# stresearch/xfr

Measured on AMD Instinct MI355X. Metric: triplet-contrastive-EBP saliency maps/sec, ResNet-101 224x224, higher is better.
Workload: dtype f32

## Files before the change

### xfr_amd/csrc/conv_gemm.hip

```cpp
#include <algorithm>
#include <atomic>
#include <mutex>
#include <vector>
#include "common.h"
#include <cstdio>
#include <cstdlib>

#include "conv_gemm_dev.h"
#include "conv_gemm_host.h"

std::atomic<long> g_conv_chain_launches[2];

namespace {

#ifndef XFR_MFM_WAVES
#define XFR_MFM_WAVES 6
#endif
#ifndef XFR_DUAL_WAVES
#define XFR_DUAL_WAVES 4
#endif
template <int TCO, int TM, int BK, int NST, int MODE, bool RELU, int CHAIN>
__global__ __launch_bounds__(NT, CHAIN == 0 ? 1 : (CHAIN == 1 ? 7 : (CHAIN == 4 ? XFR_DUAL_WAVES : XFR_MFM_WAVES))) void conv_gemm_kernel(const ConvParams p, const int n_co_tiles, const int n_m_tiles)
{
    constexpr bool ROW = TCO == 32;
// ... 673 lines not shown
        return &conv_gemm_ks_kernel<BK, NST, MODE, decltype(relu)::value, decltype(chain)::value>;
    });
}

template <int BK>
bool ks_ok(const ConvParams& p)
{
    if ((p.Cin % BK) != 0) return false;
    if (p.kh == 1 && p.kw == 1) return p.pad == 0 && p.stride <= 2;
    if (p.out_stride != 1) return false;
    return p.stride == 1 && p.tap_major == 1 && p.kh * p.kw <= 64;
}

bool is_vec_1x1(const ConvParams& p)
{
    return p.kh == 1 && p.kw == 1 && p.stride == 1 && p.pad == 0 && (p.M % 4) == 0 && p.OH == p.H && p.OW == p.W;
}

template <int BK, int NST>
bool launch_cfg_ks(const ConvParams& p, hipStream_t s)
{
    if (is_vec_1x1(p)) return launch_one_ks<BK, NST, MODE_VEC>(p, s);
    return launch_one_ks<BK, NST, MODE_TAP>(p, s);
}

template <int TCO, int TM, int BK, int NST>
bool launch_cfg(const ConvParams& p_in, hipStream_t s)
{
    ConvParams p = p_in;
    if (p.dualacc && p.kh == 1 && p.kw == 1 && p.tap_major == 0 && (p.Cin % 16) == 0) p.tap_major = 1;
    if (is_vec_1x1(p)) return launch_one<TCO, TM, BK, NST, MODE_VEC>(p, s);
    if (p.tap_major == 2) return launch_one<64, 64, 16, 4, MODE_TAP4>(p, s);
    if (p.tap_major && (p.Cin % BK) == 0) return launch_one<TCO, TM, BK, NST, MODE_TAP>(p, s);
    if (p.tap_major) return launch_one<TCO, TM, 16, 4, MODE_TAP>(p, s);
    return launch_one<TCO, TM, 16, 4, MODE_GEN>(p, s);
}

}

int conv_gemm_num_cus() { return num_cus(); }
int conv_gemm_plan_chain(ConvParams& q) { return plan_chain(q); }
void conv_gemm_warn_interpreted(const ConvParams& q) { warn_interpreted(q); }

int conv_gemm_chain_sig(const EwChain& ch)
{
    uint16_t codes[XFR_MAX_EW_STEPS];
    const int n = ew_chain_codes(ch, codes);
    if (n <= 0) return -1;
    for (int sgi = 0; sgi < kNumChainSigs; ++sgi) {
        bool same = true;
        for (int i = 0; i < XFR_MAX_EW_STEPS && same; ++i) same = kChainSigs[sgi][i] == (i < n ? codes[i] : 0);
        if (same) return sgi;
    }
    return -1;
}
int conv_gemm_num_chain_sigs() { return kNumChainSigs; }

int conv_gemm_cannot_launch(const ConvParams& p)
{
    if (p.chain.n <= 0) return 0;
    ConvParams q = p;
    return plan_chain(q);
}
const char* conv_gemm_refusal(int why)
{
    switch (why) {
        case 0: return "the convolution launch was refused without a reason";
        case 1: return "a dual (W / relu(W)) convolution launch carries a fused chain without a compiled epilogue";
        case 3: return "lean probe-forward steps and the dual-accumulator launch (ConvParams::dualacc) only exist together, behind a compiled epilogue";
        case 2: return "a fused chain with a MaxFeatureMap step (pair maximum / fan-out VJP) has no compiled epilogue and the interpreter does not run those steps";
        default: return "unknown convolution launch refusal";
    }
}

void conv_gemm_chain_launch_counts(long* compiled, long* interpreted)
{
    if (compiled) *compiled = g_conv_chain_launches[0].load();
    if (interpreted) *interpreted = g_conv_chain_launches[1].load();
}

static int pick_cfg_impl(const ConvParams& p_in, bool allow_split)
{
    ConvParams p = p_in;
    if (p.dualacc) { p.nhalves = 2; p.dualacc = 0; const int c = pick_cfg_impl(p, false); return c == CFG_ROW32 ? CFG_K16 : c; }
    if (allow_split && p.split_ok && conv_gemm_split_wanted(p)) return CFG_BF16X6;
    {
        const int rem = p.CoutTot % 64;
#ifndef XFR_NO_ROW_TILE
        if (rem > 0 && rem <= 32 && p.tap_major != 2 && p.out_stride == 1 && p.CoutTot > 32 && p.M > 64) return CFG_ROW32;
#endif
    }
    if (ks_ok<8>(p)) {
        if (p.kh == 1 && (p.stride == 2 || p.out_stride == 2 || p.as_strided)) return CFG_KS_4_4;
        if ((p.kh > 1 && p.K >= 2048) || (p.kh == 1 && (p.K == 512 || p.K >= 2048))) return CFG_KS_4_4;
    }
    const long tiles = (long)((p.CoutTot + 63) / 64) * p.nhalves * ((p.M + 63) / 64);
    if (p.K >= 1024 && tiles <= 512 && (p.tap_major ? (p.Cin % 32 == 0) : true)) return CFG_K32;
    return CFG_K16;
}
int conv_gemm_pick_cfg(const ConvParams& p_in) { return pick_cfg_impl(p_in, true); }

namespace {
struct LogRec { void* stream; int cout, nhalves, K, M, kh, chain, cfg, parts; };
std::mutex g_tune_mu;
std::atomic<int> g_tuning{0};
unsigned long long* g_stamps = nullptr;
int g_stamps_cap = 0;
int g_stamp_regions = 0, g_stamp_seq = 0;
unsigned long long* g_log = nullptr;
int g_log_cap = 0;
std::vector<LogRec> g_log_recs;
thread_local int g_last_cfg = 0;
constexpr size_t NO_LOG = (size_t)-1;

size_t tune_begin(ConvParams& p, hipStream_t s)
{
    p.stamps = nullptr;
    p.stamps_cap = 0;
    p.stamp_regions = 0;
    p.stamp_seq = 0;
    p.span = nullptr;
    size_t log_idx = NO_LOG;
    if (g_tuning.load(std::memory_order_relaxed)) {
        std::lock_guard<std::mutex> lk(g_tune_mu);
        p.stamps = g_stamps;
        p.stamps_cap = g_stamps_cap;
        p.stamp_regions = g_stamp_regions;
        p.stamp_seq = g_stamps ? g_stamp_seq++ : 0;
        if (g_log && (int)g_log_recs.size() < g_log_cap) {
            p.span = g_log + 8 * g_log_recs.size();
            log_idx = g_log_recs.size();
            g_log_recs.push_back(LogRec{(void*)s, p.CoutTot, p.dualacc ? 2 : p.nhalves, p.K, p.M, p.kh, p.chain.n, -1, 1});
        }
    }
    return log_idx;
}
void tune_ran(size_t log_idx, int cfg, int parts = 1)
{
    g_last_cfg = cfg;
    if (log_idx == NO_LOG) return;
    std::lock_guard<std::mutex> lk(g_tune_mu);
    if (log_idx < g_log_recs.size()) { g_log_recs[log_idx].cfg = cfg; g_log_recs[log_idx].parts = parts; }
}
int cfg_remap(int cfg)
{
    struct Remap { int v[32]; };
    static const Remap remap = [] {
        Remap r;
        for (int i = 0; i < 32; ++i) r.v[i] = i;
        if (const char* e = getenv("XFR_CFG_REMAP")) {
            int a = 0, b = 0, n = 0;
            while (sscanf(e, "%d:%d%n", &a, &b, &n) == 2) {
                if (a >= 0 && a < 32 && b >= 0 && b < 32) r.v[a] = b;
                e += n;
                if (*e == ',') ++e;
            }
        }
        return r;
    }();
    return (cfg >= 0 && cfg < 32) ? remap.v[cfg] : cfg;
}
}

void conv_gemm_set_stamps(unsigned long long* dev_ptr, int capacity_workgroups)
{
    std::lock_guard<std::mutex> lk(g_tune_mu);
// ... 51 lines not shown
```

### xfr_amd/csrc/conv_gemm_split.hip

```cpp
#include <algorithm>
#include <atomic>
#include <mutex>
#include <unordered_map>
#include <cstdio>
#include <cstdlib>
#include <type_traits>
#include "conv_gemm_dev.h"
#include "conv_gemm_host.h"

namespace {

typedef __bf16 v8bf __attribute__((ext_vector_type(8)));
typedef unsigned v4u __attribute__((ext_vector_type(4)));
constexpr int SP_T = 128, SP_BK = 16;
constexpr int SP_A_BYTES = 3 * 2 * SP_T * 16, SP_B_BYTES = 3 * 2 * SP_T * 16;
constexpr size_t SP_LDS = 3 * (size_t)(SP_A_BYTES + SP_B_BYTES);

typedef float v2f_t __attribute__((ext_vector_type(2)));
typedef __bf16 v2bf_t __attribute__((ext_vector_type(2)));
__device__ __forceinline__ unsigned cvt_pk_bf16(float lo, float hi)
{
    const v2f_t t = {lo, hi};
    return __builtin_bit_cast(unsigned, __builtin_convertvector(t, v2bf_t));
}
__device__ __forceinline__ void split_pair(float a, float b, unsigned& p0, unsigned& p1, unsigned& p2)
{
    p0 = cvt_pk_bf16(a, b);
    const float ra = a - __uint_as_float(p0 << 16), rb = b - __uint_as_float(p0 & 0xffff0000u);
    p1 = cvt_pk_bf16(ra, rb);
    const float sa = ra - __uint_as_float(p1 << 16), sb = rb - __uint_as_float(p1 & 0xffff0000u);
    p2 = cvt_pk_bf16(sa, sb);
}

constexpr int SPP_MAX_HALO = 64, SPP_MAX_TAPS = 25;

__host__ __device__ inline int spp_halo(const ConvParams& p) { return p.pad * p.W + p.pad; }
__host__ __device__ inline int spp_patch_len(const ConvParams& p) { return SP_T + 2 * spp_halo(p); }
inline size_t spp_lds_bytes(const ConvParams& p) { return (size_t)3 * SP_A_BYTES + (size_t)2 * 6 * (spp_patch_len(p) + 1) * 16; }

constexpr int NT8 = 512;

template <int N>
__device__ __forceinline__ void sp8_wait_barrier()
{
    asm volatile("s_waitcnt vmcnt(%0) lgkmcnt(0)\n\ts_barrier" ::"n"(N) : "memory");
}

template <bool RELU, int CHAIN, bool PATCH>
__global__ __launch_bounds__(NT8, 2) void conv_gemm_split_kernel(const ConvParams p, const uint16_t* __restrict__ ws0, const uint16_t* __restrict__ ws1,
                                                                  const int n_co_tiles, const int n_m_tiles)
{
    extern __shared__ __attribute__((aligned(16))) float smem[];
    unsigned char* lds = reinterpret_cast<unsigned char*>(smem);
    constexpr int NST = 3, D = NST - 1, XBASE = NST * SP_A_BYTES;
    const int tid = threadIdx.x, lane = tid & 63, wave8 = __builtin_amdgcn_readfirstlane(tid >> 6);
    const int wr4 = wave8 >> 1, wc = wave8 & 1;
    const int l31 = lane & 31, lhi = lane >> 5;
    const bool two_dma = wave8 < 4;
    if (wave8 < 4) stamp(p, wave8, lane, 0, 4);

    const int nparts = p.tail_s > 1 ? p.tail_s : 1;
    const int tile_lin = nparts > 1 ? (int)blockIdx.x / nparts : (int)blockIdx.x;
    const int part = (int)blockIdx.x - tile_lin * nparts;
    const int lid = xcd_remap(tile_lin, n_co_tiles * n_m_tiles);
    const int tile_m = lid / n_co_tiles;
    const int tile_co_all = lid - tile_m * n_co_tiles;
    const int n_co_half = n_co_tiles / p.nhalves;
    const int half = tile_co_all / n_co_half;
    const int tile_co = tile_co_all - half * n_co_half;
    const int co0 = tile_co * SP_T, m0 = tile_m * SP_T;
    const uint16_t* __restrict__ wsel = half ? ws1 : ws0;
    const float* __restrict__ bsel = half ? p.bias_pos : p.bias;
    float* __restrict__ osel = half ? p.out1 : p.out0;
    const int T = p.kh * p.kw, ncb = p.Cin / SP_BK, nk = p.K / SP_BK;
    const int units = PATCH ? ncb : (nk + 2) / 3, ustep = PATCH ? T : 3;
    const int ubase = units / nparts, urem = units - ubase * nparts;
    const int u0 = part * ubase + min(part, urem), u1 = u0 + ubase + (part < urem ? 1 : 0);
    const int k0 = u0 * ustep, k_end = min(u1 * ustep, nk);
    const int halo = spp_halo(p), PL = spp_patch_len(p);
    const int PS = PATCH ? (PL + 1) * 16 : SP_T * 16;
    const int XB = 6 * PS;
    const unsigned chan_bytes = (unsigned)p.in_nb * p.H * p.W * 4u;
    const __amdgpu_buffer_rsrc_t rW = __builtin_amdgcn_make_buffer_rsrc((void*)wsel, 0, n_co_half * nk * SP_A_BYTES, 0x00020000);
    const __amdgpu_buffer_rsrc_t rIn = __builtin_amdgcn_make_buffer_rsrc((void*)p.in, 0, (int)p.in_bytes, 0x00020000);
    const unsigned lds_base = (unsigned)(size_t)(__attribute__((address_space(3))) unsigned char*)(lds);

    unsigned t_voff = OOB, t_lds = 0;
    bool t_ok = false;
    int base_m = 0;
    unsigned long long tapmask = 0ull;
    const int sm = tid & 127, skq = wave8 >> 1;
    if constexpr (PATCH) {
        const int kh_ = tid >= PL ? 1 : 0, q = tid - kh_ * PL;
        const long g = (long)m0 - halo + q;
        t_ok = tid < 2 * PL;
        const bool in_row = t_ok && g >= 0 && g < (long)p.in_nb * p.H * p.W;
        t_voff = in_row ? (unsigned)g * 4u + (unsigned)(kh_ * 8) * chan_bytes : OOB;
        t_lds = lds_base + XBASE + kh_ * PS + q * 16;
    } else {
        const int m = m0 + sm;
        const bool m_ok = m < p.M;
        const int mm = m_ok ? m : 0;
        const int ohw = p.OH * p.OW;
        const int n = mm / ohw;
        const int r = mm - n * ohw;
        const int oh = r / p.OW;
        const int ow = r - oh * p.OW;
        const int ih0 = oh * p.stride - p.pad, iw0 = ow * p.stride - p.pad - p.pad_dw;
        base_m = n * p.H * p.W + ih0 * p.W + iw0;
        if (m_ok) {
            unsigned long long vw = 0ull;
            for (int dw = 0; dw < p.kw; ++dw)
                if ((unsigned)(iw0 + dw) < (unsigned)p.W) vw |= 1ull << dw;
            for (int dh = 0; dh < p.kh; ++dh)
                if ((unsigned)(ih0 + dh) < (unsigned)p.H) tapmask |= vw << (dh * p.kw);
        }
        t_lds = lds_base + XBASE + ((skq >> 1) * SP_T + sm) * 16 + (skq & 1) * 8;
    }
    int c_pos[2] = {0, 0};
    unsigned c_mask[2] = {0u, 0u};
    if constexpr (PATCH) {
#pragma unroll
        for (int j = 0; j < 2; ++j) {
            const int c = wc * 64 + j * 32 + l31, m = m0 + c;
            c_pos[j] = c + halo;
            unsigned mk = 0u;
            if (m < p.M) {
                const int ohw = p.OH * p.OW;
                const int r = m % ohw;
                const int oh = r / p.OW, ow = r - oh * p.OW;
                for (int dh = 0; dh < p.kh; ++dh)
                    for (int dw = 0; dw < p.kw; ++dw)
                        if ((unsigned)(oh + dh - p.pad) < (unsigned)p.H && (unsigned)(ow + dw - p.pad) < (unsigned)p.W) mk |= 1u << (dh * p.kw + dw);
            }
            c_mask[j] = mk;
        }
    }
    const unsigned char* a_lane = lds + (lhi * SP_T + wr4 * 32 + l31) * 16;
    const unsigned char* b_plane = lds + XBASE + lhi * PS;

    v16f acc[2], pipe[2];
#pragma unroll
    for (int j = 0; j < 2; ++j)
#pragma unroll
        for (int r = 0; r < 16; ++r) { acc[j][r] = 0.f; pipe[j][r] = 0.f; }

    auto dma = [&](int kt, int stage, int ch) {
        __builtin_amdgcn_raw_ptr_buffer_load_lds(rW, (lptr_t)(lds + stage * SP_A_BYTES + ch * 1024), 16, (ch * 1024 + lane * 16) | (kt < k_end ? 0u : OOB),
                                                 (tile_co * nk + kt) * SP_A_BYTES, 0, 0);
    };
    auto load_w = [&](int kt, int stage) {
        dma(kt, stage, wave8);
        if (two_dma) dma(kt, stage, 8 + wave8);
    };
    auto fold = [&](bool negated) {
        if (negated) { acc[0] -= pipe[0]; acc[1] -= pipe[1]; }
        else { acc[0] += pipe[0]; acc[1] += pipe[1]; }
    };
    auto mfmas = [&](const v8bf (&af)[3], const v8bf (&bf)[3][2], auto FIRST) {
        constexpr int TA[6] = {2, 1, 0, 1, 0, 0}, TB[6] = {0, 1, 2, 0, 1, 0};
        v16f zero;
#pragma unroll
        for (int r = 0; r < 16; ++r) zero[r] = 0.f;
#pragma unroll
        for (int t = 0; t < 6; ++t)
#pragma unroll
            for (int j = 0; j < 2; ++j)
                pipe[j] = __builtin_amdgcn_mfma_f32_32x32x16_bf16(af[TA[t]], bf[TB[t]][j], (t == 0 && decltype(FIRST)::value) ? zero : pipe[j], 0, 0, 0);
    };
    std::integral_constant<int, 0> S0; std::integral_constant<int, 1> S1; std::integral_constant<int, 2> S2;
    std::integral_constant<bool, true> first; std::integral_constant<bool, false> later;

    if constexpr (PATCH) {
        float xp[8];
        auto load_patch = [&](int cb) {
            const unsigned so = (unsigned)(cb * SP_BK) * chan_bytes;
#pragma unroll
            for (int i = 0; i < 8; ++i) xp[i] = __uint_as_float(__builtin_amdgcn_raw_buffer_load_b32(rIn, t_voff, so + (unsigned)i * chan_bytes, 0));
        };
        auto store_patch = [&](int buf, unsigned flip) {
            v4u q0, q1, q2;
#pragma unroll
            for (int i = 0; i < 4; ++i) {
                const float a = RELU ? fmaxf(xp[2 * i], 0.f) : xp[2 * i], b = RELU ? fmaxf(xp[2 * i + 1], 0.f) : xp[2 * i + 1];
                unsigned h0, h1, h2;
                split_pair(a, b, h0, h1, h2);
                q0[i] = h0 ^ flip; q1[i] = h1 ^ flip; q2[i] = h2 ^ flip;
            }
            if (t_ok) {
                const unsigned at = t_lds + buf * XB;
                asm volatile("ds_write_b128 %0, %1" :: "v"(at), "v"(q0));
                asm volatile("ds_write_b128 %0, %1" :: "v"(at + 2 * PS), "v"(q1));
                asm volatile("ds_write_b128 %0, %1" :: "v"(at + 4 * PS), "v"(q2));
            }
        };
        int tap = 0, cb = u0, buf = 0, shift = -halo, tdw = 0;
        bool xl_prev = false, xl_now = false;
        const bool mfma_first = wave8 < 4;
        auto load_part = [&](int kt, v8bf (&af)[3], v8bf (&bf)[3][2]) {
            const int st1 = (kt + 1) % 3, st3 = kt % 3;
            const bool more = cb + 1 < u1;
            xl_now = false;
            if (more && tap == 2) store_patch(buf ^ 1, ((cb + 1) & 1) ? 0x80008000u : 0u);
            load_w(k0 + kt + 3, kt < 0 ? 2 : st3);
            if (more && tap == 0) { load_patch(cb + 1); xl_now = true; }
            const unsigned char* As = a_lane + (kt < 0 ? 0 : st1) * SP_A_BYTES;
#pragma unroll
            for (int pc = 0; pc < 3; ++pc) af[pc] = *(const v8bf*)(As + pc * 2 * SP_T * 16);
#pragma unroll
            for (int j = 0; j < 2; ++j) {
                const int pos = ((c_mask[j] >> tap) & 1u) ? c_pos[j] + shift : PL;
                const unsigned char* Bs = b_plane + buf * XB + pos * 16;
#pragma unroll
                for (int pc = 0; pc < 3; ++pc) bf[pc][j] = *(const v8bf*)(Bs + pc * 2 * PS);
            }
            tap += 1; tdw += 1; shift += 1;
            if (tdw == p.kw) { tdw = 0; shift += p.W - p.kw; }
            if (tap == T) { tap = 0; shift = -halo; cb += 1; buf ^= 1; }
        };
        auto end_step = [&]() {
            if (xl_now || xl_prev) { if (two_dma) sp8_wait_barrier<10>(); else sp8_wait_barrier<9>(); }
            else { if (two_dma) sp8_wait_barrier<2>(); else sp8_wait_barrier<1>(); }
            xl_prev = xl_now;
        };
        auto step = [&](int kt, v8bf (&caf)[3], v8bf (&cbf)[3][2], v8bf (&naf)[3], v8bf (&nbf)[3][2], auto FIRST) {
            if (mfma_first) mfmas(caf, cbf, FIRST);
            __builtin_amdgcn_sched_barrier(0);
            load_part(kt, naf, nbf);
            __builtin_amdgcn_sched_barrier(0);
            if (!mfma_first) mfmas(caf, cbf, FIRST);
            end_step();
        };
        if (tid < 12) {
            const v4u z = {0u, 0u, 0u, 0u};
            asm volatile("ds_write_b128 %0, %1" :: "v"(lds_base + XBASE + (tid / 6) * XB + (tid % 6) * PS + PL * 16), "v"(z));
        }
        if (u1 - u0 == 1) {
            const v4u z = {0u, 0u, 0u, 0u};
            for (int i = tid; i < 6 * (PL + 1); i += NT8) asm volatile("ds_write_b128 %0, %1" :: "v"(lds_base + XBASE + XB + i * 16), "v"(z));
        }
        load_w(k0, 0);
        load_w(k0 + 1, 1);
        load_patch(u0);
        asm volatile("s_waitcnt vmcnt(0)" ::: "memory");
        store_patch(0, (u0 & 1) ? 0x80008000u : 0u);
        sp8_wait_barrier<0>();
        v8bf f0a[3], f0b[3][2], f1a[3], f1b[3][2];
        load_part(-1, f0a, f0b);
        end_step();
        if (wave8 < 4) stamp(p, wave8, lane, 1);
        int pass_in_blk = 0;
// ... 51 lines not shown
            load_w(kt + D, stD);
            load_x(kt + 3, xnew);
            const unsigned char* As = a_lane + wst * SP_A_BYTES;
            const unsigned char* Bs = b_plane + st * XB + (wc * 64 + l31) * 16;
            v8bf af[3], bf[3][2];
#pragma unroll
            for (int pc = 0; pc < 3; ++pc) {
                af[pc] = *(const v8bf*)(As + pc * 2 * SP_T * 16);
#pragma unroll
                for (int j = 0; j < 2; ++j) bf[pc][j] = *(const v8bf*)(Bs + pc * 2 * PS + j * 32 * 16);
            }
            mfmas(af, bf, FIRST);
            store_x(xcur, st1, flip);
            if (two_dma) sp8_wait_barrier<8 + 2 * (D - 1)>(); else sp8_wait_barrier<8 + (D - 1)>();
            wst = wst + 1 == NST ? 0 : wst + 1;
        };
        float x0[4], x1[4], x2[4];
        unsigned flip = (u0 & 1) ? 0x80008000u : 0u;
        load_w(k0, 0);
        load_x(k0, x0);
        asm volatile("s_waitcnt vmcnt(0)" ::: "memory");
        store_x(x0, 0, flip);
#pragma unroll
        for (int d = 1; d < D; ++d) load_w(k0 + d, d);
        load_x(k0 + 1, x0);
        load_x(k0 + 2, x1);
        if (two_dma) sp8_wait_barrier<8 + 2 * (D - 1)>(); else sp8_wait_barrier<8 + (D - 1)>();
        if (wave8 < 4) stamp(p, wave8, lane, 1);
        for (int kt = k0; kt < k_end; kt += 3) {
            const bool negated = flip != 0u;
            step(kt, S0, x0, x2, flip, first);
            step(kt + 1, S1, x1, x0, flip, later);
            flip ^= 0x80008000u;
            step(kt + 2, S2, x2, x1, flip, later);
            fold(negated);
        }
    }
    wait_vmcnt<0>();
    asm volatile("s_waitcnt lgkmcnt(0)" ::: "memory");
    if (wave8 < 4) stamp(p, wave8, lane, 2);

    if (nparts > 1) {
        constexpr int TILE_FLOATS = SP_T * SP_T;
        float* __restrict__ slab = p.tail_ws + ((long)tile_lin * nparts + part) * TILE_FLOATS + tid;
#pragma unroll
        for (int j = 0; j < 2; ++j)
#pragma unroll
            for (int r = 0; r < 16; ++r) __hip_atomic_store(slab + (j * 16 + r) * NT8, acc[j][r], __ATOMIC_RELAXED, __HIP_MEMORY_SCOPE_AGENT);
        wait_vmcnt<0>();
        __syncthreads();
        int* flag = reinterpret_cast<int*>(smem);
        if (tid == 0) {
            const unsigned old = atomicAdd(p.tail_cnt + tile_lin, 1u);
            const int last = (old == (unsigned)(nparts - 1));
            if (last) atomicExch(p.tail_cnt + tile_lin, 0u);
            *flag = last;
        }
        __syncthreads();
        const int last_part = *flag;
        __syncthreads();
        if (!last_part) {
            if (wave8 < 4) { stamp(p, wave8, lane, 3); stamp(p, wave8, lane, 4); }
            return;
        }
        const float* __restrict__ src = p.tail_ws + (long)tile_lin * nparts * TILE_FLOATS + tid;
#pragma unroll
        for (int j = 0; j < 2; ++j)
#pragma unroll
            for (int r = 0; r < 16; ++r) acc[j][r] = 0.f;
        for (int q = 0; q < nparts; ++q, src += TILE_FLOATS) {
            float v[32];
#pragma unroll
            for (int r = 0; r < 32; ++r) v[r] = __hip_atomic_load(src + r * NT8, __ATOMIC_RELAXED, __HIP_MEMORY_SCOPE_AGENT);
#pragma unroll
            for (int r = 0; r < 32; ++r) acc[r >> 4][r & 15] += v[r];
        }
    }
    if (wave8 < 4) stamp(p, wave8, lane, 3);

#pragma unroll 1
    for (int c = 0; c < 2; ++c) {
        v16f t = acc[0];
        const int wq = (wr4 & 1) * 2 + c;
        block_epilogue<CHAIN>(p, t, smem + (wave8 - wq) * (32 * 36), tid & 255, lane, wq, co0 + (wr4 >> 1) * 64, m0 + wc * 64, half, -1, 0, 1, osel, bsel, nullptr);
        acc[0] = acc[1];
    }
    if (wave8 < 4) stamp(p, wave8, lane, 4);
}

__global__ void split_pack_kernel(const float* __restrict__ w, uint16_t* __restrict__ planes, int K, int cout, int ldw, int taps)
{
    const long idx = (long)blockIdx.x * blockDim.x + threadIdx.x;
    if (idx >= (long)K * cout) return;
    const int k = (int)(idx / cout), co = (int)(idx - (long)k * cout);
    unsigned h[3];
    split_pair(w[(long)k * ldw + co], 0.f, h[0], h[1], h[2]);
    const int cin = K / taps, tap = k / cin, ci = k - tap * cin;
    const int rt = co / SP_T, r = co - rt * SP_T, kt = (ci / SP_BK) * taps + tap, kk = ci % SP_BK, nk = K / SP_BK;
#pragma unroll
    for (int q = 0; q < 3; ++q)
        planes[((((long)(rt * nk + kt) * 3 + q) * 2 + kk / 8) * SP_T + r) * 8 + kk % 8] = (uint16_t)(h[q] & 0xffffu);
}

struct SplitPack { uint16_t* planes; int K, cout, ldw, taps; };
static std::mutex g_split_mu;
static std::unordered_map<const float*, SplitPack> g_split;

bool split_patch_ok(const ConvParams& p)
{
    const int T = p.kh * p.kw;
    if (T < 5 || T > SPP_MAX_TAPS || (T % 3) != 0 || p.stride != 1 || p.tap_major != 1) return false;
    if (p.OH != p.H || p.OW != p.W || 2 * p.pad != p.kh - 1 || 2 * p.pad != p.kw - 1 || p.pad_dw != 0) return false;
    static const bool off = getenv("XFR_SPLIT_NO_PATCH") != nullptr;
    return spp_halo(p) <= SPP_MAX_HALO && !off;
}

bool split_can_run(const ConvParams& p)
{
    if (p.dualacc || p.out_stride != 1 || p.as_strided || p.co_pair > 0 || p.stride != 1) return false;
    if ((p.Cin % SP_BK) != 0 || (p.K % SP_BK) != 0 || (p.CoutTot % SP_T) != 0) return false;
    if (p.kh == 1 && p.kw == 1) return p.pad == 0;
    return p.tap_major == 1 && p.kh * p.kw <= 64;
}
struct SplitPolicy { int min_k1, min_k3, min_tiles, min_hw, max_parts, min_steps, min_cb, parts_below_hw; };
const SplitPolicy& split_policy()
{
    static const SplitPolicy pol = [] {
        SplitPolicy q{256, 1152, 128, 49, 2, 32, 4, 196};
        if (const char* e = getenv("XFR_SPLIT_MIN_K1")) q.min_k1 = atoi(e);
        if (const char* e = getenv("XFR_SPLIT_MIN_K3")) q.min_k3 = atoi(e);
        if (const char* e = getenv("XFR_SPLIT_MIN_TILES")) q.min_tiles = atoi(e);
        if (const char* e = getenv("XFR_SPLIT_MIN_HW")) q.min_hw = atoi(e);
        if (const char* e = getenv("XFR_SPLIT_MAX_PARTS")) q.max_parts = atoi(e);
        if (const char* e = getenv("XFR_SPLIT_MIN_STEPS")) q.min_steps = atoi(e);
        if (const char* e = getenv("XFR_SPLIT_MIN_CB")) q.min_cb = atoi(e);
        if (const char* e = getenv("XFR_SPLIT_PARTS_BELOW_HW")) q.parts_below_hw = atoi(e);
        return q;
    }();
    return pol;
}
bool split_layer_ok(const ConvParams& p)
{
    if (!split_can_run(p)) return false;
    if (p.OH * p.OW < split_policy().min_hw) return false;
    return p.K >= (p.kh == 1 && p.kw == 1 ? split_policy().min_k1 : split_policy().min_k3);
}
int split_pick_parts(const ConvParams& p)
{
    if (!p.tail_ws || !p.tail_cnt || p.tail_force == 1) return 1;
    const long tiles = (long)(p.CoutTot / SP_T) * p.nhalves * ((p.M + SP_T - 1) / SP_T);
    if (tiles > XFR_TAIL_MAX_TILES) return 1;
    const bool patch = split_patch_ok(p);
    const int nk = p.K / SP_BK, units = patch ? p.Cin / SP_BK : (nk + 2) / 3;
    const long fit = std::min<long>(units, (long)(p.tail_ws_bytes / ((size_t)SP_T * SP_T * sizeof(float))) / tiles);
    if (p.tail_force >= 2) return (int)std::max<long>(1, std::min<long>(p.tail_force, fit));
    const SplitPolicy& pol = split_policy();
    if (p.OH * p.OW >= pol.parts_below_hw) return 1;
    const long resident = patch ? 256 : 512;
    const int min_units = patch ? pol.min_cb : (pol.min_steps + 2) / 3;
    int S = 1;
    for (int s = 2; s <= pol.max_parts && s <= fit; ++s)
        if (tiles * s <= resident && units / s >= min_units) S = s;
    return S;
}
bool split_grid_ok(const ConvParams& p)
{
    const long tiles = (long)(p.CoutTot / SP_T) * p.nhalves * ((p.M + SP_T - 1) / SP_T);
    return tiles * split_pick_parts(p) >= split_policy().min_tiles;
}

static std::atomic<long> g_split_launches{0};
static thread_local int g_split_last_parts = 1;

const uint16_t* split_planes(const float* w, int K, int cout, int ldw, int taps, hipStream_t s)
{
    std::lock_guard<std::mutex> lk(g_split_mu);
    auto it = g_split.find(w);
    if (it != g_split.end())
        return (it->second.K == K && it->second.cout == cout && it->second.ldw == ldw && it->second.taps == taps) ? it->second.planes : nullptr;
    SplitPack sp{nullptr, K, cout, ldw, taps};
    if (hipMalloc(&sp.planes, (size_t)K * cout * 3 * sizeof(uint16_t)) != hipSuccess) {
        (void)hipGetLastError();
        sp.planes = nullptr;
        g_split[w] = sp;
        return nullptr;
    }
    const long n = (long)K * cout;
    hipLaunchKernelGGL(split_pack_kernel, dim3((unsigned)((n + 255) / 256)), dim3(256), 0, s, w, sp.planes, K, cout, ldw, taps);
    if (hipStreamSynchronize(s) != hipSuccess) { (void)hipFree(sp.planes); return nullptr; }
    g_split[w] = sp;
    return sp.planes;
}

template <bool RELU, int CHAIN>
void launch_split_inst(const ConvParams& q, const uint16_t* w0, const uint16_t* w1, int n_co, int n_m, hipStream_t s, bool patch)
{
    static std::atomic<unsigned long long> done{0ull};
    int dev = 0;
    (void)hipGetDevice(&dev);
    const unsigned long long bit = 1ull << (dev & 63);
    constexpr int PATCH_LDS_MAX = 3 * SP_A_BYTES + 2 * 6 * (SP_T + 2 * SPP_MAX_HALO + 1) * 16;
    if (!(done.load(std::memory_order_relaxed) & bit)) {
        (void)hipFuncSetAttribute((const void*)conv_gemm_split_kernel<RELU, CHAIN, false>, hipFuncAttributeMaxDynamicSharedMemorySize, (int)SP_LDS);
        (void)hipFuncSetAttribute((const void*)conv_gemm_split_kernel<RELU, CHAIN, true>, hipFuncAttributeMaxDynamicSharedMemorySize, PATCH_LDS_MAX);
        done.fetch_or(bit);
    }
    const dim3 grid(n_co * n_m * (q.tail_s > 1 ? q.tail_s : 1));
    if (patch) hipLaunchKernelGGL((conv_gemm_split_kernel<RELU, CHAIN, true>), grid, dim3(NT8), spp_lds_bytes(q), s, q, w0, w1, n_co, n_m);
    else hipLaunchKernelGGL((conv_gemm_split_kernel<RELU, CHAIN, false>), grid, dim3(NT8), SP_LDS, s, q, w0, w1, n_co, n_m);
}

bool launch_split(const ConvParams& p, hipStream_t s)
{
    if (p.force_cfg == CFG_BF16X6 ? !split_can_run(p) : !conv_gemm_split_wanted(p)) return false;
    if (p.chain.n > 0 && p.relu_in) return false;
    ConvParams q = p;
    q.tail_q = 0;
    q.tail_s = split_pick_parts(p);
    int family = p.relu_in ? -1 : 0;
    if (q.chain.n > 0) {
        if (conv_gemm_plan_chain(q)) return false;
        if (q.chain_sig >= 0 && chain_sig_is_dual(q.chain_sig)) return false;
        family = q.chain_sig < 0 ? 2 : (chain_sig_is_mfm(q.chain_sig) ? 3 : 1);
    }
    const bool patch = split_patch_ok(p);
    const int taps = patch ? p.kh * p.kw : 1;
    const uint16_t* w0 = split_planes(p.w, p.K, p.CoutTot, p.ldw, taps, s);
    const uint16_t* w1 = p.nhalves == 2 ? split_planes(p.w_pos, p.K, p.CoutTot, p.ldw, taps, s) : nullptr;
    if (!w0 || (p.nhalves == 2 && !w1)) return false;
    g_split_launches++;
    g_split_last_parts = q.tail_s;
    if (q.chain.n > 0) {
        g_conv_chain_launches[q.chain_sig >= 0 ? 0 : 1]++;
        if (q.chain_sig < 0) conv_gemm_warn_interpreted(q);
    }
    const int n_co = (p.CoutTot / SP_T) * p.nhalves;
    const int n_m = (p.M + SP_T - 1) / SP_T;
    switch (family) {
        case -1: launch_split_inst<true, 0>(q, w0, w1, n_co, n_m, s, patch); break;
        case 0: launch_split_inst<false, 0>(q, w0, w1, n_co, n_m, s, patch); break;
        case 1: launch_split_inst<false, 1>(q, w0, w1, n_co, n_m, s, patch); break;
        case 2: launch_split_inst<false, 2>(q, w0, w1, n_co, n_m, s, patch); break;
        default: launch_split_inst<false, 3>(q, w0, w1, n_co, n_m, s, patch); break;
    }
    return true;
}

}

void conv_gemm_forget_split(const void* lo, size_t bytes)
{
    std::lock_guard<std::mutex> lk(g_split_mu);
    const char* a = static_cast<const char*>(lo);
    for (auto it = g_split.begin(); it != g_split.end();) {
        const char* w = reinterpret_cast<const char*>(it->first);
        if (w >= a && w < a + bytes) {
            if (it->second.planes) (void)hipFree(it->second.planes);
            it = g_split.erase(it);
        } else ++it;
    }
}
int conv_gemm_split_covers(const ConvParams& p) { return split_layer_ok(p) ? 1 : 0; }
bool conv_gemm_presplit(const ConvParams& p, const float* w, hipStream_t s) { return split_planes(w, p.K, p.CoutTot, p.ldw, split_patch_ok(p) ? p.kh * p.kw : 1, s) != nullptr; }
bool conv_gemm_split_wanted(const ConvParams& p) { return split_layer_ok(p) && (p.split_ok == 2 || split_grid_ok(p)); }
bool conv_gemm_launch_split(const ConvParams& p, hipStream_t s) { return launch_split(p, s); }
long conv_gemm_split_launches() { return g_split_launches.load(); }
int conv_gemm_split_last_parts() { return g_split_last_parts; }
```

### xfr_amd/csrc/engine.hip

```cpp
#include "engine_internal.h"

namespace xfr {

thread_local std::string g_err;

xfr_status fail(xfr_status st, const char* fmt, ...)
{
    char buf[1024];
    va_list ap;
    va_start(ap, fmt);
    vsnprintf(buf, sizeof(buf), fmt, ap);
    va_end(ap);
    g_err = buf;
    return st;
}

static xfr_status allocate(xfr_engine* e)
{
    xfr_status st = layout_arena(e);
    if (st != XFR_OK) return st;
    HIP_TRY(hipMalloc(&e->arena, e->arena_floats * sizeof(float)));
    st = layout_workspace(e);
    if (st != XFR_OK) return st;
    const size_t B = (size_t)e->max_batch;
// ... 846 lines not shown
    xfr_status st = get_plan(e, seed_tensor, &plan);
    if (st != XFR_OK) return st;
    if (capacity < plan->n_firings) return fail(XFR_INVALID_ARG, "need room for %d kinds", plan->n_firings);
    for (int i = 0; i < plan->n_firings; ++i) kinds[i] = plan->firing_kinds[i];
    return XFR_OK;
}

xfr_status xfr_engine_set_inputs_ready(xfr_engine* e, int32_t ready)
{
    if (!e) return fail(XFR_INVALID_ARG, "null engine");
    e->inputs_ready = ready != 0;
    return XFR_OK;
}

xfr_status xfr_engine_set_trace(xfr_engine* e, int32_t enable)
{
    if (!e) return fail(XFR_INVALID_ARG, "null engine");
    e->trace_on = enable ? 1 : 0;
    return XFR_OK;
}

xfr_status xfr_engine_trace_size(xfr_engine* e, int32_t* n_firings)
{
    if (!e || !n_firings) return fail(XFR_INVALID_ARG, "null argument");
    *n_firings = e->last_trace_firings;
    return XFR_OK;
}

xfr_status xfr_engine_get_trace(xfr_engine* e, double* sums, int32_t* kinds, int32_t capacity)
{
    if (!e || !sums) return fail(XFR_INVALID_ARG, "null argument");
    const int nf = e->last_trace_firings, SB = e->last_trace_sb;
    if (capacity < nf * SB) return fail(XFR_INVALID_ARG, "trace needs %d doubles", nf * SB);
    HIP_TRY(hipSetDevice(e->device));
    HIP_TRY(hipDeviceSynchronize());
    HIP_TRY(hipMemcpy(sums, e->dbl_ws + 2 * e->max_batch, sizeof(double) * (size_t)nf * SB, hipMemcpyDeviceToHost));
    if (kinds) for (int i = 0; i < nf; ++i) kinds[i] = e->last_trace_kinds[i];
    return XFR_OK;
}

xfr_status xfr_debug_conv(const float* in_dev, const float* w_host, const float* bias_host, float* out_dev, int32_t cin, int32_t h,
                          int32_t w, int32_t nb, int32_t cout, int32_t kh, int32_t kw, int32_t stride, int32_t pad, int32_t relu_in,
                          int32_t cfg, int32_t reps, float* ms_out)
{
    if (!in_dev || !w_host || !out_dev || cin < 1 || cout < 1 || kh < 1 || kw < 1 || stride < 1 || reps < 1)
        return fail(XFR_INVALID_ARG, "xfr_debug_conv: bad arguments");
    const int khw = kh * kw, K = cin * khw;
    const int ldw = (int)align_up(cout, 128);
    const bool tap = khw > 1 && (cin % 16 == 0) && khw <= 64;
    const bool tap4 = khw > 1 && (cin == 3 || cin == 4) && khw <= 60;
    const int Kf = tap4 ? 4 * khw : K;
    std::vector<float> host(align_up(Kf, 32) * (size_t)ldw, 0.f);
    for (int co = 0; co < cout; ++co)
        for (int ci = 0; ci < cin; ++ci)
            for (int tp = 0; tp < khw; ++tp) {
                const size_t kk = tap4 ? (size_t)tp * 4 + ci : (tap ? (size_t)tp * cin + ci : (size_t)ci * khw + tp);
                host[kk * ldw + co] = w_host[((size_t)co * cin + ci) * khw + tp];
            }
    float *wd = nullptr, *bd = nullptr;
    HIP_TRY(hipMalloc(&wd, host.size() * sizeof(float)));
    HIP_TRY(hipMemcpy(wd, host.data(), host.size() * sizeof(float), hipMemcpyHostToDevice));
    if (bias_host) {
        HIP_TRY(hipMalloc(&bd, cout * sizeof(float)));
        HIP_TRY(hipMemcpy(bd, bias_host, cout * sizeof(float), hipMemcpyHostToDevice));
    }
    ConvParams p;
    memset(&p, 0, sizeof(p));
    p.in = in_dev; p.w = wd; p.bias = bd; p.out0 = out_dev;
    p.Cin = cin; p.H = h; p.W = w; p.NB = nb; p.in_nb = nb; p.out_nb = nb;
    p.kh = kh; p.kw = kw; p.stride = stride; p.pad = pad;
    p.OH = (h + 2 * pad - kh) / stride + 1; p.OW = (w + 2 * pad - kw) / stride + 1;
    p.K = Kf; p.K_logical = K; p.M = nb * p.OH * p.OW; p.CoutTot = cout; p.nhalves = 1; p.ldw = ldw;
    p.relu_in = relu_in; p.out_H = p.OH; p.out_W = p.OW; p.out_stride = 1;
    p.in_bytes = (unsigned)((size_t)cin * nb * h * w * sizeof(float));
    p.tap_major = tap4 ? 2 : (tap ? 1 : 0); p.force_cfg = cfg % 100;
    static float* tws = nullptr;
    if (!tws) {
        HIP_TRY(hipMalloc(&tws, XFR_TAIL_WS_BYTES + XFR_TAIL_MAX_TILES * sizeof(unsigned)));
        HIP_TRY(hipMemset(reinterpret_cast<char*>(tws) + XFR_TAIL_WS_BYTES, 0, XFR_TAIL_MAX_TILES * sizeof(unsigned)));
    }
    p.tail_ws = tws; p.tail_ws_bytes = XFR_TAIL_WS_BYTES;
    p.tail_cnt = reinterpret_cast<unsigned*>(reinterpret_cast<char*>(tws) + XFR_TAIL_WS_BYTES);
    p.tail_force = (cfg / 10000) % 100;
    const bool split = (cfg % 100) == CFG_BF16X6;
    hipEvent_t a, b;
    HIP_TRY(hipEventCreate(&a));
    HIP_TRY(hipEventCreate(&b));
    const int nstreams = std::max(1, std::min(4, cfg / 1000000));
    p.tail_force = (cfg / 10000) % 100;
    for (int r = 0; r < std::max(1, std::min(reps, 200)); ++r) launch_conv_gemm(p, 0);
    float ms = 0.f;
    if (nstreams == 1) {
        HIP_TRY(hipEventRecord(a, 0));
        for (int r = 0; r < reps; ++r) launch_conv_gemm(p, 0);
        HIP_TRY(hipEventRecord(b, 0));
        HIP_TRY(hipDeviceSynchronize());
        HIP_TRY(hipEventElapsedTime(&ms, a, b));
    } else {
        hipStream_t st[4];
        float* tw[4];
        ConvParams q[4];
        for (int i = 0; i < nstreams; ++i) {
            HIP_TRY(hipStreamCreateWithFlags(&st[i], hipStreamNonBlocking));
            HIP_TRY(hipMalloc(&tw[i], XFR_TAIL_WS_BYTES + XFR_TAIL_MAX_TILES * sizeof(unsigned)));
            q[i] = p;
            q[i].tail_ws = tw[i];
            q[i].tail_cnt = reinterpret_cast<unsigned*>(reinterpret_cast<char*>(tw[i]) + XFR_TAIL_WS_BYTES);
            HIP_TRY(hipMemset(q[i].tail_cnt, 0, XFR_TAIL_MAX_TILES * sizeof(unsigned)));
        }
        HIP_TRY(hipDeviceSynchronize());
        HIP_TRY(hipEventRecord(a, 0));
        for (int i = 0; i < nstreams; ++i) HIP_TRY(hipStreamWaitEvent(st[i], a, 0));
        for (int r = 0; r < reps; ++r)
            for (int i = 0; i < nstreams; ++i) launch_conv_gemm(q[i], st[i]);
        for (int i = 0; i < nstreams; ++i) {
            hipEvent_t e;
            HIP_TRY(hipEventCreateWithFlags(&e, hipEventDisableTiming));
            HIP_TRY(hipEventRecord(e, st[i]));
            HIP_TRY(hipStreamWaitEvent(0, e, 0));
            (void)hipEventDestroy(e);
        }
        HIP_TRY(hipEventRecord(b, 0));
        HIP_TRY(hipDeviceSynchronize());
        HIP_TRY(hipEventElapsedTime(&ms, a, b));
        ms /= nstreams;
        for (int i = 0; i < nstreams; ++i) { (void)hipStreamDestroy(st[i]); (void)hipFree(tw[i]); }
    }
    if (ms_out) *ms_out = ms / reps;
    (void)hipEventDestroy(a); (void)hipEventDestroy(b);
    if (split) conv_gemm_forget_split(wd, host.size() * sizeof(float));
    (void)hipFree(wd);
    if (bd) (void)hipFree(bd);
    HIP_TRY(hipGetLastError());
    return XFR_OK;
}

xfr_status xfr_debug_conv_stamps(void* stamps_dev, int32_t capacity_workgroups)
{
    if (stamps_dev && (capacity_workgroups == 0 || (capacity_workgroups < 0 && -capacity_workgroups < 256)))
        return fail(XFR_INVALID_ARG, "xfr_debug_conv_stamps: capacity must be positive (or <= -256: sampled mode)");
    conv_gemm_set_stamps(reinterpret_cast<unsigned long long*>(stamps_dev), capacity_workgroups);
    return XFR_OK;
}

xfr_status xfr_debug_conv_log(void* log_dev, int32_t capacity, const char* dump_path)
{
    if (dump_path) {
        const int n = conv_gemm_dump_log(dump_path);
        if (n < 0) return fail(XFR_HIP_ERROR, "xfr_debug_conv_log: cannot write %s", dump_path);
    }
    conv_gemm_set_log(reinterpret_cast<unsigned long long*>(log_dev), capacity);
    return XFR_OK;
}

xfr_status xfr_engine_profile_csv(xfr_engine* e, const char* path)
{
    if (!e) return fail(XFR_INVALID_ARG, "null engine");
    e->profile_csv = path ? path : "";
    return XFR_OK;
}

xfr_status xfr_chain_epilogue_stats(int64_t* compiled_launches, int64_t* interpreted_launches, int32_t* n_signatures)
{
    long c = 0, i = 0;
    conv_gemm_chain_launch_counts(&c, &i);
    if (compiled_launches) *compiled_launches = c;
    if (interpreted_launches) *interpreted_launches = i;
    if (n_signatures) *n_signatures = conv_gemm_num_chain_sigs();
    return XFR_OK;
}

xfr_status xfr_elementwise_launch_stats(int64_t* counts, int32_t capacity, int32_t* n_variants)
{
    const int n = elementwise_num_variants();
    if (n_variants) *n_variants = n;
    if (capacity < 0 || (capacity > 0 && !counts)) return fail(XFR_INVALID_ARG, "xfr_elementwise_launch_stats: bad arguments");
    for (int i = 0; i < n && i < capacity; ++i) counts[i] = elementwise_variant_launches(i);
    return XFR_OK;
}

const char* xfr_elementwise_variant_name(int32_t i) { return elementwise_variant_name(i); }

xfr_status xfr_engine_memory(xfr_engine* e, size_t* weight_bytes, size_t* workspace_bytes)
{
    if (!e) return fail(XFR_INVALID_ARG, "null engine");
    if (weight_bytes) *weight_bytes = e->arena_floats * sizeof(float);
    if (workspace_bytes) *workspace_bytes = e->ws_floats * sizeof(float) + e->idx_bytes;
    return XFR_OK;
}

xfr_status xfr_engine_set_profile(xfr_engine* e, int32_t enable)
{
    if (!e) return fail(XFR_INVALID_ARG, "null engine");
    e->profile_on = enable ? 1 : 0;
    return XFR_OK;
}

xfr_status xfr_engine_get_profile(xfr_engine* e, double* gemm_ms, int64_t* gemm_launches, double* gemm_flops)
{
    if (!e) return fail(XFR_INVALID_ARG, "null engine");
    if (gemm_ms) *gemm_ms = e->last_gemm_ms;
    if (gemm_launches) *gemm_launches = e->last_gemm_launches;
    if (gemm_flops) *gemm_flops = e->last_gemm_flops;
    return XFR_OK;
}

xfr_status xfr_engine_get_profile_by_kernel(xfr_engine* e, double* gemm_ms, int64_t* gemm_launches, double* gemm_flops)
{
    if (!e || !gemm_ms || !gemm_launches || !gemm_flops) return fail(XFR_INVALID_ARG, "null argument");
    for (int q = 0; q < 2; ++q) { gemm_ms[q] = e->fam_ms[q]; gemm_launches[q] = e->fam_launches[q]; gemm_flops[q] = e->fam_flops[q]; }
    return XFR_OK;
}

}
```

Baseline: 1598.

## Route dual-accumulator 1x1 convolutions through the bf16x6 split MFMA kernel

Adds a dual-accumulator instantiation (CHAIN 4) of the split bf16 MFMA kernel. From the already loaded input fragments it computes a second ReLU-masked set of products into extra accumulators, so lean probe-forward 1x1 convolutions can use the split path instead of the fp32 CFG_K16/K32 path. This doubles the accumulator registers and MFMA count per tile and disables tail splitting for these launches. Access is gated by an env var that defaults on, and the debug conv entry gains a lean-launch mode for testing.

```diff
diff --git a/xfr_amd/csrc/conv_gemm.hip b/xfr_amd/csrc/conv_gemm.hip
--- a/xfr_amd/csrc/conv_gemm.hip
+++ b/xfr_amd/csrc/conv_gemm.hip
@@ -779,6 +779,7 @@
 static int pick_cfg_impl(const ConvParams& p_in, bool allow_split)
 {
     ConvParams p = p_in;
+    if (p.dualacc && allow_split && p.split_ok && conv_gemm_split_wanted(p)) return CFG_BF16X6;
     if (p.dualacc) { p.nhalves = 2; p.dualacc = 0; const int c = pick_cfg_impl(p, false); return c == CFG_ROW32 ? CFG_K16 : c; }
     if (allow_split && p.split_ok && conv_gemm_split_wanted(p)) return CFG_BF16X6;
     {
diff --git a/xfr_amd/csrc/conv_gemm_split.hip b/xfr_amd/csrc/conv_gemm_split.hip
--- a/xfr_amd/csrc/conv_gemm_split.hip
+++ b/xfr_amd/csrc/conv_gemm_split.hip
@@ -46,10 +46,21 @@
     asm volatile("s_waitcnt vmcnt(%0) lgkmcnt(0)\n\ts_barrier" ::"n"(N) : "memory");
 }
 
+typedef short v8s __attribute__((ext_vector_type(8)));
+__device__ __forceinline__ void relu_pieces(const v8bf (&af)[3], v8bf (&ar)[3])
+{
+    const v8s keep = ~(__builtin_bit_cast(v8s, af[0]) >> 15);
+#pragma unroll
+    for (int pc = 0; pc < 3; ++pc) ar[pc] = __builtin_bit_cast(v8bf, (v8s)(__builtin_bit_cast(v8s, af[pc]) & keep));
+}
+
 template <bool RELU, int CHAIN, bool PATCH>
 __global__ __launch_bounds__(NT8, 2) void conv_gemm_split_kernel(const ConvParams p, const uint16_t* __restrict__ ws0, const uint16_t* __restrict__ ws1,
                                                                   const int n_co_tiles, const int n_m_tiles)
 {
+    constexpr bool DUAL = CHAIN == 4;
+    constexpr int NA = DUAL ? 4 : 2;
+    static_assert(!DUAL || (!RELU && !PATCH), "the dual-accumulator instantiation: slab mode, an input that is already clamped");
     extern __shared__ __attribute__((aligned(16))) float smem[];
     unsigned char* lds = reinterpret_cast<unsigned char*>(smem);
     constexpr int NST = 3, D = NST - 1, XBASE = NST * SP_A_BYTES;
@@ -139,9 +150,9 @@
     const unsigned char* a_lane = lds + (lhi * SP_T + wr4 * 32 + l31) * 16;
     const unsigned char* b_plane = lds + XBASE + lhi * PS;
 
-    v16f acc[2], pipe[2];
-#pragma unroll
-    for (int j = 0; j < 2; ++j)
+    v16f acc[NA], pipe[NA];
+#pragma unroll
+    for (int j = 0; j < NA; ++j)
 #pragma unroll
         for (int r = 0; r < 16; ++r) { acc[j][r] = 0.f; pipe[j][r] = 0.f; }
 
@@ -156,6 +167,10 @@
     auto fold = [&](bool negated) {
         if (negated) { acc[0] -= pipe[0]; acc[1] -= pipe[1]; }
         else { acc[0] += pipe[0]; acc[1] += pipe[1]; }
+        if constexpr (DUAL) {
+            if (negated) { acc[2] -= pipe[2]; acc[3] -= pipe[3]; }
+            else { acc[2] += pipe[2]; acc[3] += pipe[3]; }
+        }
     };
     auto mfmas = [&](const v8bf (&af)[3], const v8bf (&bf)[3][2], auto FIRST) {
         constexpr int TA[6] = {2, 1, 0, 1, 0, 0}, TB[6] = {0, 1, 2, 0, 1, 0};
@@ -167,6 +182,15 @@
 #pragma unroll
             for (int j = 0; j < 2; ++j)
                 pipe[j] = __builtin_amdgcn_mfma_f32_32x32x16_bf16(af[TA[t]], bf[TB[t]][j], (t == 0 && decltype(FIRST)::value) ? zero : pipe[j], 0, 0, 0);
+        if constexpr (DUAL) {
+            v8bf ar[3];
+            relu_pieces(af, ar);
+#pragma unroll
+            for (int t = 0; t < 6; ++t)
+#pragma unroll
+                for (int j = 0; j < 2; ++j)
+                    pipe[2 + j] = __builtin_amdgcn_mfma_f32_32x32x16_bf16(ar[TA[t]], bf[TB[t]][j], (t == 0 && decltype(FIRST)::value) ? zero : pipe[2 + j], 0, 0, 0);
+        }
     };
     std::integral_constant<int, 0> S0; std::integral_constant<int, 1> S1; std::integral_constant<int, 2> S2;
     std::integral_constant<bool, true> first; std::integral_constant<bool, false> later;
@@ -384,7 +408,13 @@
     for (int c = 0; c < 2; ++c) {
         v16f t = acc[0];
         const int wq = (wr4 & 1) * 2 + c;
-        block_epilogue<CHAIN>(p, t, smem + (wave8 - wq) * (32 * 36), tid & 255, lane, wq, co0 + (wr4 >> 1) * 64, m0 + wc * 64, half, -1, 0, 1, osel, bsel, nullptr);
+        if constexpr (DUAL) {
+            v16f tp = acc[2];
+            block_epilogue<4>(p, t, smem + (wave8 - wq) * (32 * 36), tid & 255, lane, wq, co0 + (wr4 >> 1) * 64, m0 + wc * 64, half, -1, 0, 1, osel, bsel, &tp);
+            acc[2] = acc[3];
+        } else {
+            block_epilogue<CHAIN>(p, t, smem + (wave8 - wq) * (32 * 36), tid & 255, lane, wq, co0 + (wr4 >> 1) * 64, m0 + wc * 64, half, -1, 0, 1, osel, bsel, nullptr);
+        }
         acc[0] = acc[1];
     }
     if (wave8 < 4) stamp(p, wave8, lane, 4);
@@ -417,9 +447,16 @@
     return spp_halo(p) <= SPP_MAX_HALO && !off;
 }
 
+constexpr bool SPLIT_DUAL_DEFAULT = true;
+bool split_dual_on()
+{
+    static const bool on = [] { const char* e = getenv("XFR_SPLIT_DUAL"); return e ? atoi(e) != 0 : SPLIT_DUAL_DEFAULT; }();
+    return on;
+}
 bool split_can_run(const ConvParams& p)
 {
-    if (p.dualacc || p.out_stride != 1 || p.as_strided || p.co_pair > 0 || p.stride != 1) return false;
+    if (p.out_stride != 1 || p.as_strided || p.co_pair > 0 || p.stride != 1) return false;
+    if (p.dualacc && (!split_dual_on() || p.nhalves != 1 || p.relu_in || p.chain.n == 0 || p.kh != 1 || p.kw != 1)) return false;
     if ((p.Cin % SP_BK) != 0 || (p.K % SP_BK) != 0 || (p.CoutTot % SP_T) != 0) return false;
     if (p.kh == 1 && p.kw == 1) return p.pad == 0;
     return p.tap_major == 1 && p.kh * p.kw <= 64;
@@ -449,7 +486,7 @@
 }
 int split_pick_parts(const ConvParams& p)
 {
-    if (!p.tail_ws || !p.tail_cnt || p.tail_force == 1) return 1;
+    if (!p.tail_ws || !p.tail_cnt || p.tail_force == 1 || p.dualacc) return 1;
     const long tiles = (long)(p.CoutTot / SP_T) * p.nhalves * ((p.M + SP_T - 1) / SP_T);
     if (tiles > XFR_TAIL_MAX_TILES) return 1;
     const bool patch = split_patch_ok(p);
@@ -502,14 +539,18 @@
     (void)hipGetDevice(&dev);
     const unsigned long long bit = 1ull << (dev & 63);
     constexpr int PATCH_LDS_MAX = 3 * SP_A_BYTES + 2 * 6 * (SP_T + 2 * SPP_MAX_HALO + 1) * 16;
+    constexpr bool HAS_PATCH = CHAIN != 4;
     if (!(done.load(std::memory_order_relaxed) & bit)) {
         (void)hipFuncSetAttribute((const void*)conv_gemm_split_kernel<RELU, CHAIN, false>, hipFuncAttributeMaxDynamicSharedMemorySize, (int)SP_LDS);
-        (void)hipFuncSetAttribute((const void*)conv_gemm_split_kernel<RELU, CHAIN, true>, hipFuncAttributeMaxDynamicSharedMemorySize, PATCH_LDS_MAX);
+        if constexpr (HAS_PATCH)
+            (void)hipFuncSetAttribute((const void*)conv_gemm_split_kernel<RELU, CHAIN, true>, hipFuncAttributeMaxDynamicSharedMemorySize, PATCH_LDS_MAX);
         done.fetch_or(bit);
     }
     const dim3 grid(n_co * n_m * (q.tail_s > 1 ? q.tail_s : 1));
-    if (patch) hipLaunchKernelGGL((conv_gemm_split_kernel<RELU, CHAIN, true>), grid, dim3(NT8), spp_lds_bytes(q), s, q, w0, w1, n_co, n_m);
-    else hipLaunchKernelGGL((conv_gemm_split_kernel<RELU, CHAIN, false>), grid, dim3(NT8), SP_LDS, s, q, w0, w1, n_co, n_m);
+    if constexpr (HAS_PATCH) {
+        if (patch) { hipLaunchKernelGGL((conv_gemm_split_kernel<RELU, CHAIN, true>), grid, dim3(NT8), spp_lds_bytes(q), s, q, w0, w1, n_co, n_m); return; }
+    }
+    hipLaunchKernelGGL((conv_gemm_split_kernel<RELU, CHAIN, false>), grid, dim3(NT8), SP_LDS, s, q, w0, w1, n_co, n_m);
 }
 
 bool launch_split(const ConvParams& p, hipStream_t s)
@@ -522,9 +563,9 @@
     int family = p.relu_in ? -1 : 0;
     if (q.chain.n > 0) {
         if (conv_gemm_plan_chain(q)) return false;
-        if (q.chain_sig >= 0 && chain_sig_is_dual(q.chain_sig)) return false;
-        family = q.chain_sig < 0 ? 2 : (chain_sig_is_mfm(q.chain_sig) ? 3 : 1);
-    }
+        family = q.chain_sig < 0 ? 2 : (chain_sig_is_dual(q.chain_sig) ? 4 : (chain_sig_is_mfm(q.chain_sig) ? 3 : 1));
+    }
+    if ((family == 4) != (p.dualacc != 0)) return false;
     const bool patch = split_patch_ok(p);
     const int taps = patch ? p.kh * p.kw : 1;
     const uint16_t* w0 = split_planes(p.w, p.K, p.CoutTot, p.ldw, taps, s);
@@ -543,6 +584,7 @@
         case 0: launch_split_inst<false, 0>(q, w0, w1, n_co, n_m, s, patch); break;
         case 1: launch_split_inst<false, 1>(q, w0, w1, n_co, n_m, s, patch); break;
         case 2: launch_split_inst<false, 2>(q, w0, w1, n_co, n_m, s, patch); break;
+        case 4: launch_split_inst<false, 4>(q, w0, w1, n_co, n_m, s, patch); break;
         default: launch_split_inst<false, 3>(q, w0, w1, n_co, n_m, s, patch); break;
     }
     return true;
diff --git a/xfr_amd/csrc/engine.hip b/xfr_amd/csrc/engine.hip
--- a/xfr_amd/csrc/engine.hip
+++ b/xfr_amd/csrc/engine.hip
@@ -952,6 +952,23 @@
     p.tail_ws = tws; p.tail_ws_bytes = XFR_TAIL_WS_BYTES;
     p.tail_cnt = reinterpret_cast<unsigned*>(reinterpret_cast<char*>(tws) + XFR_TAIL_WS_BYTES);
     p.tail_force = (cfg / 10000) % 100;
+    const bool lean = (cfg / 100) % 10 == 1;
+    float* affine = nullptr;
+    if (lean) {
+        if (relu_in || (p.M & 3)) return fail(XFR_INVALID_ARG, "xfr_debug_conv: a lean launch reads a clamped input and needs M %% 4 == 0");
+        std::vector<float> ab(2 * (size_t)cout, 0.f);
+        std::fill(ab.begin(), ab.begin() + cout, 1.f);
+        HIP_TRY(hipMalloc(&affine, ab.size() * sizeof(float)));
+        HIP_TRY(hipMemcpy(affine, ab.data(), ab.size() * sizeof(float), hipMemcpyHostToDevice));
+        p.dualacc = 1; p.bias_pos = bd; p.chain_B = nb; p.chain_eps = 1e-16f;
+        EwChain& ch = p.chain;
+        auto push = [&](int type) -> EwStep& { EwStep& q = ch.s[ch.n++]; memset(&q, 0, sizeof(q)); q.type = type; q.prior_sb = -1; return q; };
+        push(EW_LEAN_Q);
+        { EwStep& q = push(EW_AFFINE_C); q.p0 = affine; q.p1 = affine + cout; }
+        push(EW_RELU);
+        { EwStep& q = push(EW_LEAN_STORE); q.action = 0; q.pstore = out_dev + (size_t)cout * p.M; }
+        if (conv_gemm_cannot_launch(p)) { (void)hipFree(affine); return fail(XFR_UNSUPPORTED_LAYER, "xfr_debug_conv: the lean chain has no compiled epilogue"); }
+    }
     const bool split = (cfg % 100) == CFG_BF16X6;
     hipEvent_t a, b;
     HIP_TRY(hipEventCreate(&a));
@@ -1001,6 +1018,7 @@
     if (split) conv_gemm_forget_split(wd, host.size() * sizeof(float));
     (void)hipFree(wd);
     if (bd) (void)hipFree(bd);
+    if (affine) (void)hipFree(affine);
     HIP_TRY(hipGetLastError());
     return XFR_OK;
 }
```

New measurement: 1619 (median of 6 runs). 1.01x the previous value.
